# swami1995/diff-qp-mpc

Measured on AMD Instinct MI355X. Metric: QPs/sec (fwd+bwd), batch=4096 n=3 m=3 T=5, higher is better.
Workload: dtype f64; 1 GPU; random dense QP family R (SURVEY 8d), configs[0] shape at the BASELINE metric batch: B=4096/GPU nz=30 nineq=30 neq=15; global_batch=4096, n_state=3, n_ctrl=3, T=5, parallelism=batch-shard x1, termination=batch (the reference's batch-coupled rule, parity-safe)

## Files before the change

diff-qp-mpc_amd/csrc/dqp_r16_prims.h:

```cpp
#ifndef DQP_R16_PRIMS_H_
#define DQP_R16_PRIMS_H_
#include <hip/hip_runtime.h>
#include <math.h>

#include "dqp_common.h"

namespace dqp {
namespace r16 {

template <int CTRL> __device__ __forceinline__ double dppd(double v)
{
    return __builtin_amdgcn_update_dpp(v, v, CTRL, 0xf, 0xf, true);
}

__device__ __forceinline__ double rb(double v, int k)
{
    switch (k & 15) {
    case 0: return dppd<0x150>(v);   case 1: return dppd<0x151>(v);
    case 2: return dppd<0x152>(v);   case 3: return dppd<0x153>(v);
    case 4: return dppd<0x154>(v);   case 5: return dppd<0x155>(v);
    case 6: return dppd<0x156>(v);   case 7: return dppd<0x157>(v);
    case 8: return dppd<0x158>(v);   case 9: return dppd<0x159>(v);
    case 10: return dppd<0x15a>(v);  case 11: return dppd<0x15b>(v);
    case 12: return dppd<0x15c>(v);  case 13: return dppd<0x15d>(v);
// ... 358 lines not shown
            if (16 * s + 15 < k) continue;
            if (16 * s > k) b[s] = fma(-L[s][k], yk, b[s]);
            else b[s] = (r == lk) ? yk : fma(r > lk ? -L[s][k] : 0.0, yk, b[s]);
        }
    }
}

template <int S, int N>
__device__ __forceinline__ void tri_store(double *P, const double (&L)[S][N], int r, double *dummy)
{
#pragma unroll
    for (int s = 0; s < S; ++s) {
        const int i = r + 16 * s;
#pragma unroll
        for (int j = 0; j < N; ++j) {
            if (j > 16 * s + 15) continue;
            double *dst = (i < N && j <= i) ? P + tri(i) + j : dummy;
            *dst = L[s][j];
        }
    }
}

template <int S, int N>
__device__ __forceinline__ void tri_mv(const double *P, const double (&x)[S], double (&y)[S], int r)
{
#pragma unroll
    for (int s = 0; s < S; ++s) y[s] = 0.0;
#pragma unroll
    for (int j = 0; j < N; ++j) {
        const double xb = BC(x, j);
#pragma unroll
        for (int s = 0; s < S; ++s) {
            if (16 * s + 15 < j) continue;
            const int i = r + 16 * s;
            const int ic = i < N ? i : N - 1;
            const double v = P[tri(ic) + (j <= ic ? j : 0)];
            y[s] = fma(mask_hi(v, j <= i && i < N), xb, y[s]);
        }
    }
}

template <int S, int N>
__device__ __forceinline__ void tri_solve(const double *P, const double (&rd)[S], double (&b)[S], int r)
{
#pragma unroll
    for (int k = 0; k < N; ++k) {
        const int sk = k >> 4, lk = k & 15;
        const double yk = rb(b[sk] * rd[sk], lk);
#pragma unroll
        for (int s = 0; s < S; ++s) {
            if (16 * s + 15 < k) continue;
            const int i = r + 16 * s;
            const int ic = i < N ? i : N - 1;
            const double v = P[tri(ic) + (k <= ic ? k : 0)];
            if (16 * s > k) b[s] = fma((i < N) ? -v : 0.0, yk, b[s]);
            else b[s] = (r == lk) ? yk : fma((r > lk && i < N) ? -v : 0.0, yk, b[s]);
        }
    }
}

template <int S, int N>
__device__ __forceinline__ void tri_solve_T(const double *P, const double (&rd)[S], double (&b)[S], int r)
{
#pragma unroll
    for (int j = N - 1; j >= 0; --j) {
        const int sj = j >> 4, lj = j & 15;
        double part = 0.0;
#pragma unroll
        for (int s = 0; s < S; ++s) {
            if (16 * s + 15 <= j) continue;
            const int i = r + 16 * s;
            const int ic = i < N ? i : N - 1;
            const double v = P[tri(ic) + (j <= ic ? j : 0)];
            part = fma((i > j && i < N) ? v : 0.0, b[s], part);
        }
        const double tot = row_sum(part);
        if (r == lj) b[sj] = (b[sj] - tot) * rd[sj];
    }
}

template <int S>
__device__ __forceinline__ void vec_put(double *P, const double (&v)[S], int n, int r, double *dummy)
{
#pragma unroll
    for (int s = 0; s < S; ++s) {
        const int i = r + 16 * s;
        double *dst = i < n ? P + i : dummy;
        *dst = v[s];
    }
}
template <int S>
__device__ __forceinline__ void vec_get(const double *P, double (&v)[S], int n, int r)
{
#pragma unroll
    for (int s = 0; s < S; ++s) {
        const int i = r + 16 * s;
        const double x = P[i < n ? i : n - 1];
        v[s] = i < n ? x : 0.0;
    }
}

template <int S, int NC, bool V2>
__device__ __forceinline__ void load_rows_staged(const double *src, int nrows, double (&dst)[S][NC], int r, double *stage)
{
#pragma unroll
    for (int s = 0; s < S; ++s) {
        const int nr = nrows - 16 * s < 16 ? nrows - 16 * s : 16;
        const double *blk = src + 16 * s * NC;
        if (V2 && (reinterpret_cast<unsigned long long>(blk) & 15ull) == 0) {
            const double2 *b2 = reinterpret_cast<const double2 *>(blk);
            double2 *s2 = reinterpret_cast<double2 *>(stage);
#pragma unroll
            for (int k = 0; k < (16 * NC / 2 + 15) / 16; ++k) {
                const int e = r + 16 * k;
                if (e < nr * NC / 2) s2[e] = b2[e];
            }
            if ((nr * NC) & 1) { if (r == 0) stage[nr * NC - 1] = blk[nr * NC - 1]; }
        } else {
#pragma unroll
            for (int k = 0; k < NC; ++k) {
                const int e = r + 16 * k;
                if (e < nr * NC) stage[e] = blk[e];
            }
        }
        __syncthreads();
        const double *row = stage + (r < nr ? r : 0) * NC;
#pragma unroll
        for (int j = 0; j < NC; ++j) dst[s][j] = row[j];
        if (16 * s + 15 >= nrows) {
            const double keep = r < nr ? 1.0 : 0.0;
#pragma unroll
            for (int j = 0; j < NC; ++j) dst[s][j] *= keep;
        }
        __syncthreads();
    }
}

template <int S, int NC>
__device__ __forceinline__ void load_rows(const double *src, int nrows, double (&dst)[S][NC], int r)
{
#pragma unroll
    for (int s = 0; s < S; ++s) {
        const int i = r + 16 * s;
        const double *row = src + (i < nrows ? i : nrows - 1) * NC;
        const double keep = i < nrows ? 1.0 : 0.0;
#pragma unroll
        for (int j = 0; j < NC; ++j) dst[s][j] = row[j];
        if (16 * s + 15 >= nrows) {
#pragma unroll
            for (int j = 0; j < NC; ++j) dst[s][j] *= keep;
        }
    }
}

template <class C>
__device__ __forceinline__ void load_T(double *lds, double (&T)[C::SM][C::M],
                                       const double (&rdiag)[C::SM], const double (&dinv)[C::SM], int r)
{
    constexpr int M = C::M, SM = C::SM;
    double *Rp = lds + C::oR;
#pragma unroll
    for (int s = 0; s < SM; ++s) {
        const int i = r + 16 * s;
        double *dst = i < M ? Rp + tri(i) + i : lds + C::oDummy + r;
        *dst = rdiag[s] + dinv[s];
    }
#pragma unroll
    for (int s = 0; s < SM; ++s) {
        const int i = r + 16 * s;
        const int ic = i < M ? i : M - 1;
#pragma unroll
        for (int j = 0; j < M; ++j) {
            int off;
            if (16 * s > j) off = tri(ic) + j;
            else if (16 * s + 15 < j) off = tri(j) + ic;
            else off = (j <= ic) ? tri(ic) + j : tri(j) + ic;
            const double v = Rp[off];
            T[s][j] = (16 * s + 15 >= M) ? mask_hi(v, i < M) : v;
        }
    }
}

template <class C>
__device__ __forceinline__ void factor_T(double *lds, double (&T)[C::SM][C::M],
                                         const double (&rdiag)[C::SM], const double (&dinv)[C::SM],
                                         double (&rdu)[C::SM], int r)
{
    load_T<C>(lds, T, rdiag, dinv, r);
    lu_rows<C::SM, C::M>(T, rdu, r);
}

template <class C>
__device__ __forceinline__ void factor_T_rhs(double *lds, double (&T)[C::SM][C::M],
                                             const double (&rdiag)[C::SM], const double (&dinv)[C::SM],
                                             double (&rdu)[C::SM], double (&b)[C::SM], int r)
{
    load_T<C>(lds, T, rdiag, dinv, r);
    lu_factor_solve<C::SM, C::M, DQP_LU_FOLD_RHS != 0>(T, rdu, b, r);
}

}
}
#endif
```

diff-qp-mpc_amd/csrc/dqp_r16n.hip:

```cpp

#include "dqp_r16_prims.h"

namespace dqp {
namespace r16n {

using namespace dqp::r16;

template <int N_, int M_, int E_> struct Cfg {
    static constexpr int N = N_, M = M_, E = E_, R = N_ - E_;
    static constexpr int SN = slots(N_), SM = slots(M_), SR = slots(N_ - E_);
    static constexpr int SE = E_ > 0 ? slots(E_) : 1, EC = E_ > 0 ? E_ : 1;
    static constexpr bool PARK = slots(N_) >= 3;
#ifndef DQP_R16N_PARK_WU
#define DQP_R16N_PARK_WU 1
#endif
    static constexpr bool PARKWU = PARK || DQP_R16N_PARK_WU;
#ifndef DQP_R16N_PIN_ALL
#define DQP_R16N_PIN_ALL 1
#endif
    static constexpr bool PIN = PARK || DQP_R16N_PIN_ALL;
#ifndef DQP_R16N_SPLIT_ALL
#define DQP_R16N_SPLIT_ALL 0
#endif
    static constexpr bool SPLIT = PARK || DQP_R16N_SPLIT_ALL;
#ifndef DQP_R16N_EARLY_CTX
#define DQP_R16N_EARLY_CTX 1
#endif
    static constexpr bool EARLY = DQP_R16N_EARLY_CTX;
    static constexpr int tailsz = E_ * (N_ - E_) + E_ * (E_ - 1) / 2;
    static constexpr int oLq = 0;
    static constexpr int oTl = tri(N_);
    static constexpr int oR = oTl;
    static constexpr int shared = tailsz > tri(M_) ? tailsz : tri(M_);
    static constexpr int oCp = oTl + shared;
    static constexpr int oHp = oCp + (N_ - E_);
    static constexpr int oQv = oHp + M_;
    static constexpr int oBw = oQv + N_;
    static constexpr int oBs = oBw + (N_ - E_), oBz = oBs + M_, oBc = oBz + M_;
    static constexpr int oDummy = oBc + 2;
    static constexpr int ldsQP = oDummy + 16;
    static constexpr int ldsQPpad = (ldsQP + 1) & ~1;
#ifndef DQP_R16N_STAGED
#define DQP_R16N_STAGED 0
#endif
    static constexpr bool STAGED = DQP_R16N_STAGED && 16 * N_ <= ldsQP - oTl;
    __host__ __device__ static constexpr int toff(int k) { return k * (N_ - E_) + k * (k - 1) / 2; }
    static constexpr int wTl = 0, wLq = tailsz, wG = wLq + tri(N_), wU = wG + M_ * N_;
    static constexpr int wTau = wU + E_ * E_, wRdu = wTau + E_, wRdq = wRdu + E_;
    static constexpr int wXy = wRdq + N_, wPy = wXy + E_, wW1 = wPy + E_, wDl = wW1 + E_;
    static constexpr int wsQP = wDl + 1;
    static constexpr int snapDim = (N_ - E_) + 2 * M_ + 2;
};

#define DQP_PHASE_FENCE() asm volatile("" ::: "memory")
__device__ __forceinline__ void pin(double &x) { asm volatile("" : "+v"(x) : : "memory"); }
__device__ __forceinline__ const double *relabel(const double *p)
{
    asm volatile("" : "+v"(p));
    return p;
}

template <class C> struct State {
    double Gh[C::SM][C::N];
    double LqZ[C::SN][C::R];
    double Ah[C::SE][C::N];
    double tau[C::SE];
    double rdu1[C::SE];
    double xy[C::SE];
    double py[C::SE];
    double w1[C::SE];
    double rdq[C::SN];
    double rdiag[C::SM];
    int status;
};

template <class C>
__device__ __forceinline__ void shift_down(const double (&vn)[C::SN], double (&ve)[C::SE], int r)
{
#pragma unroll
    for (int s = 0; s < C::SE; ++s) ve[s] = 0.0;
#pragma unroll
    for (int e = 0; e < C::E; ++e) {
        const double t = BC(vn, C::R + e);
        if (r == (e & 15)) ve[e >> 4] = t;
    }
}
template <class C>
__device__ __forceinline__ void shift_up(const double (&ve)[C::SE], double (&vn)[C::SN], int r)
{
#pragma unroll
    for (int e = 0; e < C::E; ++e) {
        const double t = BC(ve, e);
        if (r == ((C::R + e) & 15)) vn[(C::R + e) >> 4] = t;
    }
}

template <class C>
__device__ __forceinline__ void reflect1(const double *lds, const double (&tau)[C::SE],
                                         double (&v)[C::SN], int k, int r)
{
    const int ck = C::R + k;
    const double *tl = lds + C::oTl + C::toff(k);
    double ud[C::SN], dot = 0.0;
#pragma unroll
    for (int s = 0; s < C::SN; ++s) {
        if (16 * s > ck) { ud[s] = 0.0; continue; }
        const int c = r + 16 * s;
        const double t = tl[c < ck ? c : 0];
        ud[s] = c < ck ? t : (c == ck ? 1.0 : 0.0);
        dot = fma(ud[s], v[s], dot);
    }
    const double tw = BC(tau, k) * row_sum(dot);
#pragma unroll
    for (int s = 0; s < C::SN; ++s)
        if (16 * s <= ck) v[s] = fma(-tw, ud[s], v[s]);
}
template <class C>
__device__ __forceinline__ void apply_QfT(const double *lds, const double (&tau)[C::SE],
                                          double (&v)[C::SN], int r)
{
#pragma unroll
    for (int k = C::E - 1; k >= 0; --k) reflect1<C>(lds, tau, v, k, r);
}
template <class C>
__device__ __forceinline__ void apply_Qf(const double *lds, const double (&tau)[C::SE],
                                         double (&v)[C::SN], int r)
{
#pragma unroll
    for (int k = 0; k < C::E; ++k) reflect1<C>(lds, tau, v, k, r);
}

template <class C>
__device__ __forceinline__ void solve_UT(const State<C> &st, double (&t)[C::SE], int r)
{
#pragma unroll
    for (int j = 0; j < C::E; ++j) {
        const int sj = j >> 4, lj = j & 15;
        double part = 0.0;
#pragma unroll
        for (int s = 0; s < C::SE; ++s) {
            if (16 * s >= j) continue;
            const int k = r + 16 * s;
            part = fma(k < j ? st.Ah[s][C::R + j] : 0.0, t[s], part);
        }
        const double tot = row_sum(part);
        if (r == lj) t[sj] = (t[sj] - tot) * st.rdu1[sj];
    }
}

template <class C>
__device__ __forceinline__ void mul_Gz(const State<C> &st, const double (&v)[C::SR], double (&y)[C::SM])
{
#pragma unroll
    for (int s = 0; s < C::SM; ++s) y[s] = 0.0;
#pragma unroll
    for (int t = 0; t < C::R; ++t) {
        const double vb = BC(v, t);
#pragma unroll
        for (int s = 0; s < C::SM; ++s) y[s] = fma(st.Gh[s][t], vb, y[s]);
    }
}
template <class C>
__device__ __forceinline__ void mul_GzT(const State<C> &st, const double (&v)[C::SM], double (&y)[C::SR], int r)
{
#pragma unroll
    for (int g = 0; g < C::SR; ++g) {
        double p[16];
#pragma unroll
        for (int k = 0; k < 16; ++k) {
            const int c = 16 * g + k;
            if (c < C::R) {
                double a = st.Gh[0][c < C::R ? c : 0] * v[0];
#pragma unroll
                for (int s = 1; s < C::SM; ++s) a = fma(st.Gh[s][c < C::R ? c : 0], v[s], a);
                p[k] = a;
            } else {
                p[k] = 0.0;
            }
        }
        y[g] = reduce_scatter16(p, r);
    }
}
template <class C>
__device__ __forceinline__ void mul_WT(const State<C> &st, const double (&v)[C::SM], double (&y)[C::SE], int r)
{
#pragma unroll
    for (int g = 0; g < C::SE; ++g) {
        double p[16];
#pragma unroll
        for (int k = 0; k < 16; ++k) {
            const int e = 16 * g + k;
            if (e < C::E) {
                double a = st.Gh[0][C::R + (e < C::E ? e : 0)] * v[0];
#pragma unroll
                for (int s = 1; s < C::SM; ++s) a = fma(st.Gh[s][C::R + (e < C::E ? e : 0)], v[s], a);
                p[k] = a;
            } else {
                p[k] = 0.0;
// ... 65 lines not shown
template <int COUNT>
__device__ __forceinline__ void ctx_fetch(const double *src, CtxRegs<COUNT> &t, int r)
{
#pragma unroll
    for (int k = 0; k < (COUNT + 15) / 16; ++k) {
        const int e = r + 16 * k;
        t.v[k] = src[(16 * k + 15 < COUNT || e < COUNT) ? e : COUNT - 1];
    }
}
template <int COUNT>
__device__ __forceinline__ void ctx_stash(double *dst, const CtxRegs<COUNT> &t, int r)
{
#pragma unroll
    for (int k = 0; k < (COUNT + 15) / 16; ++k) {
        const int e = r + 16 * k;
        if (16 * k + 15 < COUNT || e < COUNT) dst[e] = t.v[k];
    }
}
template <int COUNT>
__device__ __forceinline__ void lds_to_ctx(const double *src, double *dst, int r)
{
    CtxRegs<COUNT> t;
    ctx_fetch<COUNT>(src, t, r);
    ctx_stash<COUNT>(dst, t, r);
}

template <class C>
__device__ __forceinline__ void park_GU(double *ws, const State<C> &st, int r)
{
    constexpr int N = C::N, M = C::M, E = C::E, R = C::R;
#pragma unroll
    for (int s = 0; s < C::SM; ++s) {
        const int i = r + 16 * s;
        if (i < M) {
#pragma unroll
            for (int c = 0; c < N; ++c) ws[C::wG + c * M + i] = st.Gh[s][c];
        }
    }
#pragma unroll
    for (int s = 0; s < C::SE; ++s) {
        const int k = r + 16 * s;
        if (k < E) {
#pragma unroll
            for (int e = 0; e < E; ++e) ws[C::wU + e * E + k] = st.Ah[s][R + e];
            ws[C::wTau + k] = st.tau[s];
            ws[C::wRdu + k] = st.rdu1[s];
        }
    }
}
template <class C>
__device__ __forceinline__ void unpark_WU(const double *ws, State<C> &st, int r)
{
    constexpr int M = C::M, E = C::E, R = C::R;
#pragma unroll
    for (int s = 0; s < C::SM; ++s) {
        const int i = r + 16 * s, ic = i < M ? i : M - 1;
#pragma unroll
        for (int e = 0; e < E; ++e) {
            const double v = ws[C::wG + (R + e) * M + ic];
            st.Gh[s][R + e] = i < M ? v : 0.0;
        }
    }
#pragma unroll
    for (int s = 0; s < C::SE; ++s) {
        const int k = r + 16 * s, kc = k < E ? k : E - 1;
#pragma unroll
        for (int e = 0; e < E; ++e) {
            const double v = ws[C::wU + e * E + kc];
            st.Ah[s][R + e] = k < E ? v : 0.0;
        }
    }
}

#ifdef DQP_SETUP_STOP
template <int K, class C> __device__ __forceinline__ double stop_sum(const State<C> &st)
{
    double a = 0.0;
#pragma unroll
    for (int s = 0; s < C::SN; ++s) a += st.rdq[s];
    if (K >= 2 || K == 0) {
#pragma unroll
        for (int s = 0; s < C::SM; ++s)
#pragma unroll
            for (int c = 0; c < C::N; ++c) a += st.Gh[s][c];
#pragma unroll
        for (int s = 0; s < C::SE; ++s)
#pragma unroll
            for (int c = 0; c < C::N; ++c) a += st.Ah[s][c];
    }
    if (K >= 3 || K == 0) {
#pragma unroll
        for (int s = 0; s < C::SE; ++s) a += st.tau[s] + st.rdu1[s] + st.xy[s];
    }
    if (K >= 4 || K == 0) {
#pragma unroll
        for (int s = 0; s < C::SE; ++s) a += st.py[s] + st.w1[s];
    }
    if (K >= 5 || K == 0) {
#pragma unroll
        for (int s = 0; s < C::SN; ++s)
#pragma unroll
            for (int c = 0; c < C::R; ++c) a += st.LqZ[s][c];
    }
    if (K >= 15) {
#pragma unroll
        for (int s = 0; s < C::SM; ++s) a += st.rdiag[s];
    }
    return a;
}
#endif

template <class C>
__device__ __forceinline__ void setup(const KParams &P, long long qp, int r, double *lds, State<C> &st)
{
    constexpr int N = C::N, M = C::M, E = C::E, R = C::R;
    constexpr int SN = C::SN, SM = C::SM, SE = C::SE, SR = C::SR;
    double *dummy = lds + C::oDummy + r;
    st.status = DQP_STATUS_OK;
    double p0[SN], h0[SM], b0[SE];
    const bool mpc = P.mC != nullptr;
    if (mpc) {
        const int n = P.mn, m = P.mm, nt = n + m, T = P.mT;
#pragma unroll
        for (int s = 0; s < SN; ++s) {
            const int i = r + 16 * s, ic = i < N ? i : N - 1, t = ic / nt;
            const double v = P.mc[((long long)t * P.B + qp) * nt + (ic - t * nt)];
            p0[s] = i < N ? v : 0.0;
        }
#pragma unroll
        for (int s = 0; s < SM; ++s) {
            const int i = r + 16 * s, k = (i < T * m ? i : i - T * m), kc = k < T * m ? k : 0, t = kc / m, ju = kc - t * m;
            const long long at = qp * mpc_bound_stride_b(P) + t * mpc_bound_stride_t(P) + ju;
            const double v = i < T * m ? P.muu[at] : -P.mul[at];
            h0[s] = i < M ? v : 0.0;
        }
#pragma unroll
        for (int s = 0; s < SE; ++s) {
            const int e = r + 16 * s, ec = e < E ? e : (E > 0 ? E - 1 : 0), t = ec / n, j = ec - t * n;
            const double v = t < T - 1 ? -P.mf[((long long)t * P.B + qp) * n + j] : P.mx0[qp * n + j];
            b0[s] = (E > 0 && e < E) ? v : 0.0;
        }
    } else {
#pragma unroll
        for (int s = 0; s < SN; ++s) p0[s] = (r + 16 * s < N) ? P.p[qp * P.sp + r + 16 * s] : 0.0;
#pragma unroll
        for (int s = 0; s < SM; ++s) h0[s] = (r + 16 * s < M) ? P.h[qp * P.sh + r + 16 * s] : 0.0;
#pragma unroll
        for (int s = 0; s < SE; ++s) b0[s] = (E > 0 && r + 16 * s < E) ? P.b[qp * P.sb + r + 16 * s] : 0.0;
    }
    {
        double Lq[SN][N];
        if (mpc) mpc_rows_Q<SN, N>(P, qp, Lq, r);
        else if (C::STAGED) load_rows_staged<SN, N, (N * N) % 2 == 0>(P.Q + qp * P.sQ, N, Lq, r, lds + C::oTl);
        else load_rows<SN, N>(P.Q + qp * P.sQ, N, Lq, r);
        if (!chol_rows<SN, N>(Lq, st.rdq, r)) st.status = DQP_STATUS_Q_NOT_PD;
        tri_store<SN, N>(lds + C::oLq, Lq, r, dummy);
    }
    __syncthreads();
    if (C::EARLY) {
        double *ws = P.workspace + qp * (long long)C::wsQP;
        lds_to_ctx<tri(N)>(lds + C::oLq, ws + C::wLq, r);
#pragma unroll
        for (int s = 0; s < SN; ++s)
            if (r + 16 * s < N) ws[C::wRdq + r + 16 * s] = st.rdq[s];
    }
    __builtin_amdgcn_sched_barrier(0);
    DQP_PHASE_FENCE();
    STAMP(P, 1);

    if (mpc) {
        if (!C::SPLIT) mpc_rows_G<SM, N>(P, M, st.Gh, r);
        if (E > 0) mpc_rows_A<SE, N>(P, qp, E, st.Ah, r);
    } else {
        if (C::STAGED) {
            if (!C::SPLIT) load_rows_staged<SM, N, (M * N) % 2 == 0>(P.G + qp * P.sG, M, st.Gh, r, lds + C::oTl);
            if (E > 0) load_rows_staged<SE, N, (C::EC * N) % 2 == 0>(P.A + qp * P.sA, E, st.Ah, r, lds + C::oTl);
        } else {
            if (!C::SPLIT) load_rows<SM, N>(P.G + qp * P.sG, M, st.Gh, r);
            if (E > 0) load_rows<SE, N>(P.A + qp * P.sA, E, st.Ah, r);
        }
    }
    {
        const double *Lp = lds + C::oLq;
#pragma unroll
        for (int j = 0; j < N; ++j) {
#pragma unroll
            for (int k = 0; k < j; ++k) {
                const double ljk = Lp[tri(j) + k];
                if (!C::SPLIT) {
#pragma unroll
                    for (int s = 0; s < SM; ++s) st.Gh[s][j] = fma(-st.Gh[s][k], ljk, st.Gh[s][j]);
                }
                if (E > 0) {
#pragma unroll
                    for (int s = 0; s < SE; ++s) st.Ah[s][j] = fma(-st.Ah[s][k], ljk, st.Ah[s][j]);
                }
            }
            const double rj = BC(st.rdq, j);
            if (!C::SPLIT) {
#pragma unroll
                for (int s = 0; s < SM; ++s) st.Gh[s][j] *= rj;
            }
            if (E > 0) {
#pragma unroll
                for (int s = 0; s < SE; ++s) st.Ah[s][j] *= rj;
            }
            if (C::PIN) {
#pragma unroll
                for (int s = 0; s < SE; ++s) pin(st.Ah[s][j]);
                if (!C::SPLIT) {
#pragma unroll
                    for (int s = 0; s < SM; ++s) pin(st.Gh[s][j]);
                }
            }
            __builtin_amdgcn_sched_barrier(0);
        }
    }
    __builtin_amdgcn_sched_barrier(0);
    DQP_PHASE_FENCE();
    STAMP(P, 2);

#pragma unroll
    for (int s = 0; s < SE; ++s) { st.tau[s] = 0.0; st.rdu1[s] = 0.0; st.xy[s] = 0.0; st.py[s] = 0.0; st.w1[s] = 0.0; }

    if (E > 0) {
        double nmax = 0.0;
#pragma unroll
        for (int k = E - 1; k >= 0; --k) {
            const int sk = k >> 4, lk = k & 15, ck = R + k;
#ifdef DQP_STAMPS_C
            if (k < 15) { STAMPC(P, k); }
#endif
            double u[N];
            double nrm2 = 0.0;
#pragma unroll
            for (int c = 0; c <= ck; ++c) {
                u[c] = rb(st.Ah[sk][c], lk);
                nrm2 = fma(u[c], u[c], nrm2);
            }
            if (!(nrm2 > 1e-26 * nmax)) { if (st.status == DQP_STATUS_OK) st.status = DQP_STATUS_A_RANK_DEF; nrm2 = 1.0; }
            nmax = fmax(nmax, nrm2);
            const double vk = u[ck];
            const double alpha = -copysign(sqrt(nrm2), vk);
            const double uck = vk - alpha;
            const double iu = frcp(uck);
            const double tauk = uck * uck * frcp(nrm2 - alpha * vk);
            double *tl = lds + C::oTl + C::toff(k);
            if (C::PIN) {
#pragma unroll
                for (int c = 0; c < ck; ++c) u[c] *= iu;
                if (r == 0) {
#pragma unroll
                    for (int c = 0; c < ck; ++c) tl[c] = u[c];
                }
            } else {
#pragma unroll
                for (int c = 0; c < ck; ++c) {
                    u[c] *= iu;
                    double *dst = (r == 0) ? tl + c : dummy;
                    *dst = u[c];
                }
            }
            if (r == lk) { st.tau[sk] = tauk; st.rdu1[sk] = frcp(alpha); }
#pragma unroll
            for (int s = 0; s < SE; ++s) {
                if (16 * s > k) continue;
                double w = st.Ah[s][ck];
#pragma unroll
                for (int c = 0; c < ck; ++c) w = fma(st.Ah[s][c], u[c], w);
                double tw = tauk * w;
                if (16 * s + 15 >= k) tw = (r + 16 * s < k) ? tw : 0.0;
#pragma unroll
                for (int c = 0; c < ck; ++c) st.Ah[s][c] = fma(-tw, u[c], st.Ah[s][c]);
                st.Ah[s][ck] -= tw;
            }
            if (r == lk) st.Ah[sk][ck] = alpha;
            if (!C::SPLIT) {
#pragma unroll
                for (int s = 0; s < SM; ++s) {
                    double w = st.Gh[s][ck];
#pragma unroll
                    for (int c = 0; c < ck; ++c) w = fma(st.Gh[s][c], u[c], w);
                    const double tw = tauk * w;
#pragma unroll
                    for (int c = 0; c < ck; ++c) st.Gh[s][c] = fma(-tw, u[c], st.Gh[s][c]);
                    st.Gh[s][ck] -= tw;
                }
            }
            if (C::PIN) {
#pragma unroll
                for (int s = 0; s < SE; ++s) pin(st.Ah[s][ck]);
                if (!C::SPLIT) {
#pragma unroll
                    for (int s = 0; s < SM; ++s) pin(st.Gh[s][ck]);
                }
            }
        }
#ifdef DQP_STAMPS_C
        STAMPC(P, 15);
#endif
        __syncthreads();
        __builtin_amdgcn_sched_barrier(0);
        if (C::EARLY) {
            double *ws = P.workspace + qp * (long long)C::wsQP;
            lds_to_ctx<C::tailsz>(lds + C::oTl, ws + C::wTl, r);
        }
        DQP_PHASE_FENCE();

        {
            double b[SE];
#pragma unroll
            for (int s = 0; s < SE; ++s) b[s] = b0[s];
#pragma unroll
            for (int j = E - 1; j >= 0; --j) {
                const int sj = j >> 4, lj = j & 15;
                const double xj = rb(b[sj] * st.rdu1[sj], lj);
#pragma unroll
                for (int s = 0; s < SE; ++s) {
                    if (16 * s > j) continue;
                    const int k = r + 16 * s;
                    b[s] = (k == j) ? xj : fma(k < j ? -st.Ah[s][R + j] : 0.0, xj, b[s]);
                }
            }
#pragma unroll
            for (int s = 0; s < SE; ++s) st.xy[s] = b[s];
        }
    }
    __builtin_amdgcn_sched_barrier(0);
    DQP_PHASE_FENCE();
// ... 353 lines not shown
            s_[s] = -z[s];
            ms = fmin(ms, inM[s] ? s_[s] : INFINITY);
            mz = fmin(mz, inM[s] ? z[s] : INFINITY);
        }
        ms = row_min(ms); mz = row_min(mz);
#pragma unroll
        for (int s = 0; s < SM; ++s) {
            if (ms < 0.0 && inM[s]) s_[s] -= ms - 1.0;
            if (mz < 0.0 && inM[s]) z[s] -= mz - 1.0;
        }
        delta = mz < 0.0 ? 1.0 - mz : 0.0;
        if (r == 0) P.workspace[qp * (long long)C::wsQP + C::wDl] = delta;
    }

    double gz[SR];
    mul_GzT<C>(st, z, gz, r);
    STAMP(P, 6);
    double best = INFINITY, bestc = 1.0;
    bool have_best = false, done = false;
    int nNot = 0, iters = 0;

    if (maxIter > 0) for (int it = 0;; ++it) {
        double rw[SR], rz[SM];
        {
            double cp[SR], hp[SM], gw[SM];
            vec_get<SR>(lds + C::oCp, cp, R, r);
            vec_get<SM>(lds + C::oHp, hp, M, r);
            mul_Gz<C>(st, w, gw);
#pragma unroll
            for (int s = 0; s < SR; ++s) rw[s] = inR[s] ? w[s] + cp[s] + gz[s] : 0.0;
#pragma unroll
            for (int s = 0; s < SM; ++s) rz[s] = inM[s] ? gw[s] + s_[s] - hp[s] : 0.0;
        }
        double sz = 0.0, nz2 = 0.0;
#pragma unroll
        for (int s = 0; s < SM; ++s) { sz = fma(s_[s], z[s], sz); nz2 = fma(rz[s], rz[s], nz2); }
        double nx2 = rx_norm2_partial<C>(st, lds, rw, cc * delta, r);
        sz = row_sum(sz); nz2 = row_sum(nz2); nx2 = row_sum(nx2);
        const double mu = fabs(sz * (1.0 / M));
        const double resid = sqrt(nz2) + sqrt(nx2) + M * mu;
        if (!done) {
            iters = it + 1;
            if (!have_best || resid < best) {
                nNot = 0; have_best = true; best = resid; bestc = cc;
                vec_put<SR>(lds + C::oBw, w, R, r, dummy);
                vec_put<SM>(lds + C::oBs, s_, M, r, dummy);
                vec_put<SM>(lds + C::oBz, z, M, r, dummy);
                if (P.snap && live) {
                    double *sp = P.snap + ((long long)it * P.B + qp) * C::snapDim;
#pragma unroll
                    for (int s = 0; s < SR; ++s)
                        if (inR[s]) sp[r + 16 * s] = w[s];
#pragma unroll
                    for (int s = 0; s < SM; ++s)
                        if (inM[s]) { sp[R + r + 16 * s] = s_[s]; sp[R + M + r + 16 * s] = z[s]; }
                    if (r == 0) sp[R + 2 * M] = cc;
                }
            } else {
                nNot += 1;
            }
            if (batch) {
                if (P.hist && r == 0 && live) hist_put(P, qp, it, resid, mu);
                done = !(fabs(resid) < INFINITY);
            } else if ((nNot >= P.notImprovedLim && best < P.stallTol) || best < P.eps || mu > 1e32 ||
                       !(fabs(resid) < INFINITY))
                done = true;
        }
        if (__builtin_amdgcn_ballot_w64(!done) == 0 || it + 1 >= maxIter) break;
        if (it == 1) STAMP(P, 9);

        double dza[SM], dsa[SM];
        {
            double gu[SM];
            mul_Gz<C>(st, rw, gu);
#pragma unroll
            for (int s = 0; s < SM; ++s) dza[s] = rz[s] - s_[s] - gu[s];
        }
        __builtin_amdgcn_sched_barrier(0);
        double dinv[SM];
#pragma unroll
        for (int s = 0; s < SM; ++s) dinv[s] = inM[s] ? s_[s] * frcp(z[s]) : 0.0;
        factor_T_rhs<C>(lds, T, st.rdiag, dinv, rdu, dza, r);
        if (it == 1) STAMP(P, 10);
        if (it == 1) STAMP(P, 11);
        double rzv[SM], rsv[SM];
#pragma unroll
        for (int s = 0; s < SM; ++s) {
            rzv[s] = inM[s] ? frcp(z[s]) : 0.0;
            rsv[s] = inM[s] ? frcp(s_[s]) : 0.0;
        }
        double tm = 0.0;
#pragma unroll
        for (int s = 0; s < SM; ++s) {
            dsa[s] = (-z[s] - dza[s]) * dinv[s];
            tm = fmax(tm, fmax(-dza[s] * rzv[s], -dsa[s] * rsv[s]));
        }
        bool zero_step = false;
        if (strict) {
#pragma unroll
            for (int s = 0; s < SM; ++s) zero_step |= inM[s] && (dza[s] == 0.0 || dsa[s] == 0.0);
        }
        double alpha = frcp(fmax(row_max(tm), 1.0));
        double t3 = 0.0;
#pragma unroll
        for (int s = 0; s < SM; ++s)
            t3 = fma(fma(alpha, dsa[s], s_[s]), fma(alpha, dza[s], z[s]), t3);
        t3 = row_sum(t3);
        double sig = t3 / sz;
        sig = sig * sig * sig;
        double rsc[SM], dzc[SM], dz[SM], ds[SM];
#pragma unroll
        for (int s = 0; s < SM; ++s) {
            rsc[s] = fma(dsa[s], dza[s], -mu * sig) * rsv[s];
            dzc[s] = -rsc[s] * dinv[s];
        }
        lu_solve<SM, M>(T, rdu, dzc, r);
        if (it == 1) STAMP(P, 12);
        tm = 0.0;
#pragma unroll
        for (int s = 0; s < SM; ++s) {
            dz[s] = dza[s] + dzc[s];
            ds[s] = fma(-rsc[s] - dzc[s], dinv[s], dsa[s]);
            tm = fmax(tm, fmax(-dz[s] * rzv[s], -ds[s] * rsv[s]));
        }
        if (strict) {
#pragma unroll
            for (int s = 0; s < SM; ++s) zero_step |= inM[s] && (dz[s] == 0.0 || ds[s] == 0.0);
            if ((__builtin_amdgcn_ballot_w64(zero_step) >> (lane & 48)) & 0xffffull) done = true;
        }
        __builtin_amdgcn_sched_barrier(0);
        double gtd[SR];
        mul_GzT<C>(st, dz, gtd, r);
        alpha = frcp(fmax(row_max(tm) * (1.0 / 0.999), 1.0));
        if (!done) {
#pragma unroll
            for (int s = 0; s < SR; ++s) {
                w[s] = fma(alpha, -rw[s] - gtd[s], w[s]);
                gz[s] = fma(alpha, gtd[s], gz[s]);
            }
#pragma unroll
            for (int s = 0; s < SM; ++s) { s_[s] = fma(alpha, ds[s], s_[s]); z[s] = fma(alpha, dz[s], z[s]); }
            cc *= (1.0 - alpha);
        }
        if (it == 1) STAMP(P, 13);
        if (it == 0) STAMP(P, 8);
    }
    STAMP(P, 7);

    if (P.hist && r == 0 && live) hist_fill(P, qp, iters);
    epilogue<C>(P, qp, r, lds, st, bestc, delta, iters, best, live, true);
    STAMP(P, 14);
}

template <class C>
__device__ __forceinline__ void load_ctx(const KParams &P, long long qp, int r, double *lds, State<C> &st)
{
    constexpr int N = C::N, M = C::M, E = C::E, R = C::R;
    constexpr int SN = C::SN, SM = C::SM, SE = C::SE;
    st.status = DQP_STATUS_OK;
    {
        const double *ws = P.workspace + qp * (long long)C::wsQP;
        CtxRegs<C::tailsz> tl;
        CtxRegs<tri(N)> lq;
        ctx_fetch<C::tailsz>(ws + C::wTl, tl, r);
        ctx_fetch<tri(N)>(ws + C::wLq, lq, r);
        ctx_stash<C::tailsz>(lds + C::oTl, tl, r);
        ctx_stash<tri(N)>(lds + C::oLq, lq, r);
#pragma unroll
        for (int s = 0; s < SM; ++s) {
            const int i = r + 16 * s, ic = i < M ? i : M - 1;
#pragma unroll
            for (int c = 0; c < N; ++c) {
                const double v = ws[C::wG + c * M + ic];
                st.Gh[s][c] = (16 * s + 15 >= M) ? mask_hi(v, i < M) : v;
            }
        }
#pragma unroll
        for (int s = 0; s < SE; ++s) {
            const int k = r + 16 * s, kc = k < E ? k : E - 1;
#pragma unroll
            for (int c = 0; c < N; ++c) st.Ah[s][c] = 0.0;
#pragma unroll
            for (int e = 0; e < E; ++e) {
                const double v = ws[C::wU + e * E + kc];
                st.Ah[s][R + e] = k < E ? v : 0.0;
            }
            const double t = ws[C::wTau + kc], u = ws[C::wRdu + kc];
            st.tau[s] = k < E ? t : 0.0;
            st.rdu1[s] = k < E ? u : 0.0;
        }
#pragma unroll
        for (int s = 0; s < SN; ++s) {
            const int i = r + 16 * s;
            const double v = ws[C::wRdq + (i < N ? i : N - 1)];
            st.rdq[s] = i < N ? v : 0.0;
        }
    }
}

template <class C>
__global__ __launch_bounds__(64) void finish_kernel(KParams P)
{
    constexpr int M = C::M, E = C::E, R = C::R;
    constexpr int SM = C::SM, SE = C::SE, SR = C::SR;
    extern __shared__ __attribute__((aligned(16))) double sm[];
    const int lane = threadIdx.x, r = lane & 15, qrow = lane >> 4;
    long long qp = (long long)blockIdx.x * 4 + qrow;
    bool live = qp < P.B;
    if (!live) qp = P.B - 1;
    live = live && term_flagged(P, qp);
    if (__builtin_amdgcn_ballot_w64(live) == 0) return;
    const int cap = min(P.maxIter, P.cap[0]);
    double *lds = sm + qrow * C::ldsQPpad;
    double *dummy = lds + C::oDummy + r;
    State<C> st;
    load_ctx<C>(P, qp, r, lds, st);
    const double *ws = P.workspace + qp * (long long)C::wsQP;
#pragma unroll
    for (int s = 0; s < SE; ++s) {
        const int k = r + 16 * s, kc = k < E ? k : (E > 0 ? E - 1 : 0);
        const double a = ws[C::wXy + kc], b = ws[C::wPy + kc], c = ws[C::wW1 + kc];
        st.xy[s] = (E > 0 && k < E) ? a : 0.0;
        st.py[s] = (E > 0 && k < E) ? b : 0.0;
        st.w1[s] = (E > 0 && k < E) ? c : 0.0;
    }
    const double delta = ws[C::wDl];
    const double2 *h = reinterpret_cast<const double2 *>(P.histIn) + qp;
    double hv[64];
#pragma unroll
    for (int it = 0; it < 64; ++it) hv[it] = h[(long long)(it < cap ? it : 0) * P.B].x;
    double best = hv[0];
    int arg = 0;
#pragma unroll
    for (int it = 1; it < 64; ++it)
        if (it < cap && hv[it] < best) { best = hv[it]; arg = it; }
    const double *sp = P.snap + ((long long)arg * P.B + qp) * C::snapDim;
    double bw[SR], bs[SM], bz[SM];
#pragma unroll
    for (int s = 0; s < SR; ++s) { const int i = r + 16 * s; const double v = sp[i < R ? i : 0]; bw[s] = i < R ? v : 0.0; }
#pragma unroll
    for (int s = 0; s < SM; ++s) {
        const int i = r + 16 * s, ic = i < M ? i : 0;
        const double a = sp[R + ic], b = sp[R + M + ic];
        bs[s] = i < M ? a : 0.0;
        bz[s] = i < M ? b : 0.0;
    }
    const double bestc = sp[R + 2 * M];
    vec_put<SR>(lds + C::oBw, bw, R, r, dummy);
    vec_put<SM>(lds + C::oBs, bs, M, r, dummy);
    vec_put<SM>(lds + C::oBz, bz, M, r, dummy);
    st.status = P.info ? P.info[2 * qp] : DQP_STATUS_OK;
    epilogue<C>(P, qp, r, lds, st, bestc, delta, cap, best, live, false);
}

template <class C>
__global__ __launch_bounds__(64) void backward_kernel(KParams P)
{
    constexpr int N = C::N, M = C::M, E = C::E, R = C::R;
    constexpr int SN = C::SN, SM = C::SM, SE = C::SE, SR = C::SR;
    extern __shared__ __attribute__((aligned(16))) double sm[];
    const int lane = threadIdx.x, r = lane & 15, qrow = lane >> 4;
    long long qp = (long long)blockIdx.x * 4 + qrow;
    const bool live = qp < P.B;
    if (!live) qp = P.B - 1;
    double *lds = sm + qrow * C::ldsQPpad;

    State<C> st;
    load_ctx<C>(P, qp, r, lds, st);
    __syncthreads();

    bool inN[SN], inM[SM], inE[SE];
#pragma unroll
    for (int s = 0; s < SN; ++s) inN[s] = r + 16 * s < N;
#pragma unroll
    for (int s = 0; s < SM; ++s) inM[s] = r + 16 * s < M;
#pragma unroll
    for (int s = 0; s < SE; ++s) inE[s] = r + 16 * s < E;

    double zh[SN], g[SN], lam[SM], dinv[SM], nu[SE];
#pragma unroll
    for (int s = 0; s < SN; ++s) {
        zh[s] = inN[s] ? P.zin[qp * N + r + 16 * s] : 0.0;
        g[s] = inN[s] ? P.gin[qp * N + r + 16 * s] : 0.0;
    }
#pragma unroll
    for (int s = 0; s < SM; ++s) {
        lam[s] = inM[s] ? P.lamin[qp * M + r + 16 * s] : 0.0;
        const double sl = inM[s] ? P.slackin[qp * M + r + 16 * s] : 1.0;
        if (P.flags & DQP_FLAG_DENSE_BACKWARD) dinv[s] = inM[s] ? sl / lam[s] : 0.0;
        else dinv[s] = inM[s] ? fmax(sl, 1e-8) / fmax(lam[s], 1e-8) : 0.0;
    }
#pragma unroll
    for (int s = 0; s < SE; ++s) nu[s] = (E > 0 && inE[s]) ? P.nuin[qp * E + r + 16 * s] : 0.0;

    tri_solve<SN, N>(lds + C::oLq, st.rdq, g, r);
    double gy[SE];
#pragma unroll
    for (int s = 0; s < SE; ++s) gy[s] = 0.0;
    if (E > 0) {
        apply_QfT<C>(lds, st.tau, g, r);
        shift_down<C>(g, gy, r);
    }
    double gz[SR];
#pragma unroll
    for (int s = 0; s < SR; ++s) gz[s] = (r + 16 * s < R) ? g[s] : 0.0;

    double dlam[SM];
    mul_Gz<C>(st, gz, dlam);
#pragma unroll
    for (int s = 0; s < SM; ++s) dlam[s] = -dlam[s];
    __builtin_amdgcn_sched_barrier(0);
    {
        double T[SM][M], rdu[SM];
#pragma unroll
        for (int j = 0; j < M; ++j) {
            const int sj = j >> 4, lj = j & 15;
            double acc[SM];
#pragma unroll
            for (int s = 0; s < SM; ++s) acc[s] = (r + 16 * s == j) ? dinv[s] : 0.0;
#pragma unroll
            for (int c = 0; c < R; ++c) {
                const double gb = rb(st.Gh[sj][c], lj);
#pragma unroll
                for (int s = 0; s < SM; ++s) acc[s] = fma(st.Gh[s][c], gb, acc[s]);
            }
#pragma unroll
            for (int s = 0; s < SM; ++s) T[s][j] = acc[s];
            __builtin_amdgcn_sched_barrier(0);
        }
        lu_factor_solve<SM, M, DQP_LU_FOLD_RHS != 0>(T, rdu, dlam, r);
    }
    __builtin_amdgcn_sched_barrier(0);
    double dxh[SN], dnu[SE];
    {
        double gtd[SR];
        mul_GzT<C>(st, dlam, gtd, r);
#pragma unroll
        for (int s = 0; s < SN; ++s) dxh[s] = (s < SR && r + 16 * s < R) ? -(gz[s < SR ? s : 0] + gtd[s < SR ? s : 0]) : 0.0;
    }
#pragma unroll
    for (int s = 0; s < SE; ++s) dnu[s] = 0.0;
    if (E > 0) {
        apply_Qf<C>(lds, st.tau, dxh, r);
        double wz[SE];
        mul_WT<C>(st, dlam, wz, r);
#pragma unroll
        for (int s = 0; s < SE; ++s) dnu[s] = inE[s] ? -(gy[s] + wz[s]) : 0.0;
        solve_UT<C>(st, dnu, r);
    }
    tri_solve_T<SN, N>(lds + C::oLq, st.rdq, dxh, r);

    if (!live) return;
    if (P.mdc || P.mdC || P.mdF || P.mdf || P.mdx0) {
        const int n = P.mn, m = P.mm, nt = n + m, T = P.mT;
        const long long Bq = P.B;
        int tl[SN], jl[SN];
#pragma unroll
        for (int s = 0; s < SN; ++s) { const int c = r + 16 * s; tl[s] = c / nt; jl[s] = c - tl[s] * nt; }
        if (P.mdc) {
#pragma unroll
            for (int s = 0; s < SN; ++s)
                if (inN[s]) P.mdc[((long long)tl[s] * Bq + qp) * nt + jl[s]] = dxh[s];
        }
        if (P.mdC) {
            int ti = 0, ji = 0;
#pragma unroll
            for (int i = 0; i < N; ++i) {
                const double dxi = BC(dxh, i), zi = BC(zh, i);
#pragma unroll
                for (int s = 0; s < SN; ++s)
                    if (inN[s] && tl[s] == ti)
                        P.mdC[(((long long)ti * Bq + qp) * nt + ji) * nt + jl[s]] = 0.5 * (dxi * zh[s] + zi * dxh[s]);
                if (++ji == nt) { ji = 0; ++ti; }
            }
        }
        if (E > 0) {
            int te = 0, je = 0;
#pragma unroll
            for (int e = 0; e < E; ++e) {
                const double dni = BC(dnu, e), ni = BC(nu, e);
                if (te < T - 1) {
                    if (P.mdF) {
#pragma unroll
                        for (int s = 0; s < SN; ++s)
                            if (inN[s] && tl[s] == te)
                                P.mdF[(((long long)te * Bq + qp) * n + je) * nt + jl[s]] = dni * zh[s] + ni * dxh[s];
                    }
                    if (P.mdf && r == 0) P.mdf[((long long)te * Bq + qp) * n + je] = dni;
                } else if (P.mdx0 && r == 0) {
                    P.mdx0[qp * n + je] = -dni;
                }
                if (++je == n) { je = 0; ++te; }
            }
        }
        if (r == 0 && P.info) { P.info[2 * qp] = st.status; P.info[2 * qp + 1] = 0; }
        return;
    }
#pragma unroll
    for (int s = 0; s < SN; ++s)
        if (P.dp && inN[s]) P.dp[qp * N + r + 16 * s] = dxh[s];
#pragma unroll
    for (int s = 0; s < SM; ++s)
        if (P.dh && inM[s]) P.dh[qp * M + r + 16 * s] = -dlam[s];
    if (E > 0) {
#pragma unroll
        for (int s = 0; s < SE; ++s)
            if (P.db && inE[s]) P.db[qp * E + r + 16 * s] = -dnu[s];
    }
    if (P.dQ) {
        double *o = P.dQ + qp * N * N;
#pragma unroll
        for (int i = 0; i < N; ++i) {
            const double dxi = BC(dxh, i), zi = BC(zh, i);
#pragma unroll
            for (int s = 0; s < SN; ++s)
                if (inN[s]) o[i * N + r + 16 * s] = 0.5 * (dxi * zh[s] + zi * dxh[s]);
        }
    }
    if (P.dG) {
        double *o = P.dG + qp * M * N;
#pragma unroll
        for (int i = 0; i < M; ++i) {
            const double dli = BC(dlam, i), li = BC(lam, i);
#pragma unroll
            for (int s = 0; s < SN; ++s)
                if (inN[s]) o[i * N + r + 16 * s] = dli * zh[s] + li * dxh[s];
        }
    }
    if (P.dA && E > 0) {
        double *o = P.dA + qp * E * N;
#pragma unroll
        for (int i = 0; i < E; ++i) {
            const double dni = BC(dnu, i), ni = BC(nu, i);
#pragma unroll
            for (int s = 0; s < SN; ++s)
                if (inN[s]) o[i * N + r + 16 * s] = dni * zh[s] + ni * dxh[s];
        }
    }
    if (r == 0 && P.info) { P.info[2 * qp] = st.status; P.info[2 * qp + 1] = 0; }
}

template <class C, class K>
int launch(K kernel, const KParams &P, void *stream)
{
    const size_t lds = (size_t)4 * C::ldsQPpad * sizeof(double);
    if (lds > 64 * 1024 &&
        hipFuncSetAttribute(reinterpret_cast<const void *>(kernel),
                            hipFuncAttributeMaxDynamicSharedMemorySize, (int)lds) != hipSuccess)
        return DQP_ERR_LAUNCH;
    const int blocks = (P.B + 3) / 4;
    DQP_LAUNCH(kernel, dim3(blocks), dim3(64), lds, (hipStream_t)stream, P);
    return hipGetLastError() == hipSuccess ? DQP_OK : DQP_ERR_LAUNCH;
}

}

#if !defined(DQP_R16_N) || !defined(DQP_R16_M) || !defined(DQP_R16_E)
#error "compile with -DDQP_R16_N=.. -DDQP_R16_M=.. -DDQP_R16_E=.."
#endif
#define DQP_CAT2(a, n, m, e) a##n##_##m##_##e
#define DQP_CAT(a, n, m, e) DQP_CAT2(a, n, m, e)

#ifndef DQP_R16_BWD
int DQP_CAT(r16n_forward_, DQP_R16_N, DQP_R16_M, DQP_R16_E)(const KParams &P, void *stream)
{
    using C = r16n::Cfg<DQP_R16_N, DQP_R16_M, DQP_R16_E>;
    if (P.cap && P.snap && P.histIn) return r16n::launch<C>(r16n::finish_kernel<C>, P, stream);
    return r16n::launch<C>(r16n::forward_kernel<C>, P, stream);
}
#else
int DQP_CAT(r16n_backward_, DQP_R16_N, DQP_R16_M, DQP_R16_E)(const KParams &P, void *stream)
{
    using C = r16n::Cfg<DQP_R16_N, DQP_R16_M, DQP_R16_E>;
    return r16n::launch<C>(r16n::backward_kernel<C>, P, stream);
}
#endif

}
```

Before: 17.51 million QPs/sec.

## Issue G/A and context loads early to overlap memory latency with compute

In the forward context setup, G and A rows are now loaded right after Q rows, so their memory latency overlaps the Cholesky factorisation, and masking is applied later. In the backward kernel, the workspace context loads (triangular factors, G columns, U, tau, rdu) are split into issue and finish stages. They are issued alongside the per-QP input loads, and masking and LDS stashing are deferred until just before each piece is consumed. This aims to hide global-load latency, at the cost of higher register pressure and more complex barrier and fence ordering.

```diff
diff --git a/diff-qp-mpc_amd/csrc/dqp_r16_prims.h b/diff-qp-mpc_amd/csrc/dqp_r16_prims.h
--- a/diff-qp-mpc_amd/csrc/dqp_r16_prims.h
+++ b/diff-qp-mpc_amd/csrc/dqp_r16_prims.h
@@ -534,6 +534,29 @@
         }
     }
 }
+template <int S, int NC>
+__device__ __forceinline__ void load_rows_issue(const double *src, int nrows, double (&dst)[S][NC], int r)
+{
+#pragma unroll
+    for (int s = 0; s < S; ++s) {
+        const int i = r + 16 * s;
+        const double *row = src + (i < nrows ? i : nrows - 1) * NC;
+#pragma unroll
+        for (int j = 0; j < NC; ++j) dst[s][j] = row[j];
+    }
+}
+template <int S, int NC>
+__device__ __forceinline__ void load_rows_mask(int nrows, double (&dst)[S][NC], int r)
+{
+#pragma unroll
+    for (int s = 0; s < S; ++s) {
+        const double keep = r + 16 * s < nrows ? 1.0 : 0.0;
+        if (16 * s + 15 >= nrows) {
+#pragma unroll
+            for (int j = 0; j < NC; ++j) dst[s][j] *= keep;
+        }
+    }
+}
 
 template <class C>
 __device__ __forceinline__ void load_T(double *lds, double (&T)[C::SM][C::M],
diff --git a/diff-qp-mpc_amd/csrc/dqp_r16n.hip b/diff-qp-mpc_amd/csrc/dqp_r16n.hip
--- a/diff-qp-mpc_amd/csrc/dqp_r16n.hip
+++ b/diff-qp-mpc_amd/csrc/dqp_r16n.hip
@@ -44,6 +44,10 @@
 #define DQP_R16N_STAGED 0
 #endif
     static constexpr bool STAGED = DQP_R16N_STAGED && 16 * N_ <= ldsQP - oTl;
+#ifndef DQP_R16N_EARLY_GA
+#define DQP_R16N_EARLY_GA 1
+#endif
+    static constexpr bool EARLYGA = DQP_R16N_EARLY_GA && !SPLIT && !STAGED;
     __host__ __device__ static constexpr int toff(int k) { return k * (N_ - E_) + k * (k - 1) / 2; }
     static constexpr int wTl = 0, wLq = tailsz, wG = wLq + tri(N_), wU = wG + M_ * N_;
     static constexpr int wTau = wU + E_ * E_, wRdu = wTau + E_, wRdq = wRdu + E_;
@@ -415,7 +419,13 @@
         double Lq[SN][N];
         if (mpc) mpc_rows_Q<SN, N>(P, qp, Lq, r);
         else if (C::STAGED) load_rows_staged<SN, N, (N * N) % 2 == 0>(P.Q + qp * P.sQ, N, Lq, r, lds + C::oTl);
-        else load_rows<SN, N>(P.Q + qp * P.sQ, N, Lq, r);
+        else {
+            load_rows<SN, N>(P.Q + qp * P.sQ, N, Lq, r);
+            if (C::EARLYGA) {
+                load_rows_issue<SM, N>(P.G + qp * P.sG, M, st.Gh, r);
+                if (E > 0) load_rows_issue<SE, N>(P.A + qp * P.sA, E, st.Ah, r);
+            }
+        }
         if (!chol_rows<SN, N>(Lq, st.rdq, r)) st.status = DQP_STATUS_Q_NOT_PD;
         tri_store<SN, N>(lds + C::oLq, Lq, r, dummy);
     }
@@ -438,6 +448,9 @@
         if (C::STAGED) {
             if (!C::SPLIT) load_rows_staged<SM, N, (M * N) % 2 == 0>(P.G + qp * P.sG, M, st.Gh, r, lds + C::oTl);
             if (E > 0) load_rows_staged<SE, N, (C::EC * N) % 2 == 0>(P.A + qp * P.sA, E, st.Ah, r, lds + C::oTl);
+        } else if (C::EARLYGA) {
+            load_rows_mask<SM, N>(M, st.Gh, r);
+            if (E > 0) load_rows_mask<SE, N>(E, st.Ah, r);
         } else {
             if (!C::SPLIT) load_rows<SM, N>(P.G + qp * P.sG, M, st.Gh, r);
             if (E > 0) load_rows<SE, N>(P.A + qp * P.sA, E, st.Ah, r);
@@ -1097,50 +1110,101 @@
     STAMP(P, 14);
 }
 
+template <class C> struct CtxA {
+    CtxRegs<C::tailsz> tl;
+    CtxRegs<tri(C::N)> lq;
+};
+#ifndef DQP_R16N_BWD_ORDERED_CTX
+#define DQP_R16N_BWD_ORDERED_CTX 1
+#endif
+template <class C>
+__device__ __forceinline__ void ctx_issue_a(const double *ws, int r, CtxA<C> &a, State<C> &st)
+{
+    ctx_fetch<C::tailsz>(ws + C::wTl, a.tl, r);
+    ctx_fetch<tri(C::N)>(ws + C::wLq, a.lq, r);
+#pragma unroll
+    for (int s = 0; s < C::SN; ++s) {
+        const int i = r + 16 * s;
+        st.rdq[s] = ws[C::wRdq + (i < C::N ? i : C::N - 1)];
+    }
+#pragma unroll
+    for (int s = 0; s < C::SE; ++s) {
+        const int k = r + 16 * s;
+        st.tau[s] = ws[C::wTau + (k < C::E ? k : C::E - 1)];
+    }
+}
+template <class C>
+__device__ __forceinline__ void ctx_finish_a(double *lds, int r, const CtxA<C> &a, State<C> &st)
+{
+    ctx_stash<C::tailsz>(lds + C::oTl, a.tl, r);
+    ctx_stash<tri(C::N)>(lds + C::oLq, a.lq, r);
+#pragma unroll
+    for (int s = 0; s < C::SN; ++s) st.rdq[s] = r + 16 * s < C::N ? st.rdq[s] : 0.0;
+#pragma unroll
+    for (int s = 0; s < C::SE; ++s) st.tau[s] = r + 16 * s < C::E ? st.tau[s] : 0.0;
+}
+template <class C, int C0, int C1>
+__device__ __forceinline__ void ctx_issue_G(const double *ws, int r, State<C> &st)
+{
+#pragma unroll
+    for (int s = 0; s < C::SM; ++s) {
+        const int i = r + 16 * s, ic = i < C::M ? i : C::M - 1;
+#pragma unroll
+        for (int c = C0; c < C1; ++c) st.Gh[s][c] = ws[C::wG + c * C::M + ic];
+    }
+}
+template <class C, int C0, int C1>
+__device__ __forceinline__ void ctx_finish_G(int r, State<C> &st)
+{
+#pragma unroll
+    for (int s = 0; s < C::SM; ++s) {
+        if (16 * s + 15 < C::M) continue;
+#pragma unroll
+        for (int c = C0; c < C1; ++c) st.Gh[s][c] = mask_hi(st.Gh[s][c], r + 16 * s < C::M);
+    }
+}
+template <class C>
+__device__ __forceinline__ void ctx_issue_c(const double *ws, int r, State<C> &st)
+{
+    ctx_issue_G<C, C::R, C::N>(ws, r, st);
+#pragma unroll
+    for (int s = 0; s < C::SE; ++s) {
+        const int k = r + 16 * s, kc = k < C::E ? k : C::E - 1;
+#pragma unroll
+        for (int e = 0; e < C::E; ++e) st.Ah[s][C::R + e] = ws[C::wU + e * C::E + kc];
+        st.rdu1[s] = ws[C::wRdu + kc];
+    }
+}
+template <class C>
+__device__ __forceinline__ void ctx_finish_c(int r, State<C> &st)
+{
+    ctx_finish_G<C, C::R, C::N>(r, st);
+#pragma unroll
+    for (int s = 0; s < C::SE; ++s) {
+        const bool in = r + 16 * s < C::E;
+#pragma unroll
+        for (int e = 0; e < C::E; ++e) st.Ah[s][C::R + e] = in ? st.Ah[s][C::R + e] : 0.0;
+        st.rdu1[s] = in ? st.rdu1[s] : 0.0;
+    }
+}
 template <class C>
 __device__ __forceinline__ void load_ctx(const KParams &P, long long qp, int r, double *lds, State<C> &st)
 {
-    constexpr int N = C::N, M = C::M, E = C::E, R = C::R;
-    constexpr int SN = C::SN, SM = C::SM, SE = C::SE;
     st.status = DQP_STATUS_OK;
+    const double *ws = P.workspace + qp * (long long)C::wsQP;
+#pragma unroll
+    for (int s = 0; s < C::SE; ++s)
+#pragma unroll
+        for (int c = 0; c < C::R; ++c) st.Ah[s][c] = 0.0;
     {
-        const double *ws = P.workspace + qp * (long long)C::wsQP;
-        CtxRegs<C::tailsz> tl;
-        CtxRegs<tri(N)> lq;
-        ctx_fetch<C::tailsz>(ws + C::wTl, tl, r);
-        ctx_fetch<tri(N)>(ws + C::wLq, lq, r);
-        ctx_stash<C::tailsz>(lds + C::oTl, tl, r);
-        ctx_stash<tri(N)>(lds + C::oLq, lq, r);
-#pragma unroll
-        for (int s = 0; s < SM; ++s) {
-            const int i = r + 16 * s, ic = i < M ? i : M - 1;
-#pragma unroll
-            for (int c = 0; c < N; ++c) {
-                const double v = ws[C::wG + c * M + ic];
-                st.Gh[s][c] = (16 * s + 15 >= M) ? mask_hi(v, i < M) : v;
-            }
-        }
-#pragma unroll
-        for (int s = 0; s < SE; ++s) {
-            const int k = r + 16 * s, kc = k < E ? k : E - 1;
-#pragma unroll
-            for (int c = 0; c < N; ++c) st.Ah[s][c] = 0.0;
-#pragma unroll
-            for (int e = 0; e < E; ++e) {
-                const double v = ws[C::wU + e * E + kc];
-                st.Ah[s][R + e] = k < E ? v : 0.0;
-            }
-            const double t = ws[C::wTau + kc], u = ws[C::wRdu + kc];
-            st.tau[s] = k < E ? t : 0.0;
-            st.rdu1[s] = k < E ? u : 0.0;
-        }
-#pragma unroll
-        for (int s = 0; s < SN; ++s) {
-            const int i = r + 16 * s;
-            const double v = ws[C::wRdq + (i < N ? i : N - 1)];
-            st.rdq[s] = i < N ? v : 0.0;
-        }
-    }
+        CtxA<C> a;
+        ctx_issue_a<C>(ws, r, a, st);
+        ctx_finish_a<C>(lds, r, a, st);
+    }
+    ctx_issue_G<C, 0, C::R>(ws, r, st);
+    ctx_issue_c<C>(ws, r, st);
+    ctx_finish_G<C, 0, C::R>(r, st);
+    ctx_finish_c<C>(r, st);
 }
 
 template <class C>
@@ -1210,19 +1274,30 @@
     if (!live) qp = P.B - 1;
     double *lds = sm + qrow * C::ldsQPpad;
 
+    bool inN[SN], inM[SM], inE[SE];
+#pragma unroll
+    for (int s = 0; s < SN; ++s) inN[s] = r + 16 * s < N;
+#pragma unroll
+    for (int s = 0; s < SM; ++s) inM[s] = r + 16 * s < M;
+#pragma unroll
+    for (int s = 0; s < SE; ++s) inE[s] = r + 16 * s < E;
+
+    constexpr bool ORD = DQP_R16N_BWD_ORDERED_CTX && !C::PARK;
     State<C> st;
-    load_ctx<C>(P, qp, r, lds, st);
-    __syncthreads();
-
-    bool inN[SN], inM[SM], inE[SE];
-#pragma unroll
-    for (int s = 0; s < SN; ++s) inN[s] = r + 16 * s < N;
-#pragma unroll
-    for (int s = 0; s < SM; ++s) inM[s] = r + 16 * s < M;
-#pragma unroll
-    for (int s = 0; s < SE; ++s) inE[s] = r + 16 * s < E;
-
-    double zh[SN], g[SN], lam[SM], dinv[SM], nu[SE];
+    const double *ws = P.workspace + qp * (long long)C::wsQP;
+    double zh[SN], g[SN], lam[SM], sl[SM], dinv[SM], nu[SE];
+    if (ORD) {
+        st.status = DQP_STATUS_OK;
+#pragma unroll
+        for (int s = 0; s < SE; ++s)
+#pragma unroll
+            for (int c = 0; c < R; ++c) st.Ah[s][c] = 0.0;
+    } else {
+        load_ctx<C>(P, qp, r, lds, st);
+        __syncthreads();
+    }
+    CtxA<C> ca;
+    if (ORD) ctx_issue_a<C>(ws, r, ca, st);
 #pragma unroll
     for (int s = 0; s < SN; ++s) {
         zh[s] = inN[s] ? P.zin[qp * N + r + 16 * s] : 0.0;
@@ -1231,12 +1306,24 @@
 #pragma unroll
     for (int s = 0; s < SM; ++s) {
         lam[s] = inM[s] ? P.lamin[qp * M + r + 16 * s] : 0.0;
-        const double sl = inM[s] ? P.slackin[qp * M + r + 16 * s] : 1.0;
-        if (P.flags & DQP_FLAG_DENSE_BACKWARD) dinv[s] = inM[s] ? sl / lam[s] : 0.0;
-        else dinv[s] = inM[s] ? fmax(sl, 1e-8) / fmax(lam[s], 1e-8) : 0.0;
+        sl[s] = inM[s] ? P.slackin[qp * M + r + 16 * s] : 1.0;
     }
 #pragma unroll
     for (int s = 0; s < SE; ++s) nu[s] = (E > 0 && inE[s]) ? P.nuin[qp * E + r + 16 * s] : 0.0;
+    if (ORD) {
+        ctx_issue_G<C, 0, R>(ws, r, st);
+        ctx_issue_c<C>(ws, r, st);
+        __builtin_amdgcn_sched_barrier(0);
+        ctx_finish_a<C>(lds, r, ca, st);
+        __builtin_amdgcn_fence(__ATOMIC_RELEASE, "workgroup", "local");
+        __builtin_amdgcn_s_barrier();
+        __builtin_amdgcn_fence(__ATOMIC_ACQUIRE, "workgroup", "local");
+    }
+#pragma unroll
+    for (int s = 0; s < SM; ++s) {
+        if (P.flags & DQP_FLAG_DENSE_BACKWARD) dinv[s] = inM[s] ? sl[s] / lam[s] : 0.0;
+        else dinv[s] = inM[s] ? fmax(sl[s], 1e-8) / fmax(lam[s], 1e-8) : 0.0;
+    }
 
     tri_solve<SN, N>(lds + C::oLq, st.rdq, g, r);
     double gy[SE];
@@ -1251,6 +1338,12 @@
     for (int s = 0; s < SR; ++s) gz[s] = (r + 16 * s < R) ? g[s] : 0.0;
 
     double dlam[SM];
+    if (ORD) {
+#pragma unroll
+        for (int s = 0; s < SR; ++s) pin(gz[s]);
+        __builtin_amdgcn_sched_barrier(0);
+        ctx_finish_G<C, 0, R>(r, st);
+    }
     mul_Gz<C>(st, gz, dlam);
 #pragma unroll
     for (int s = 0; s < SM; ++s) dlam[s] = -dlam[s];
@@ -1287,6 +1380,10 @@
     for (int s = 0; s < SE; ++s) dnu[s] = 0.0;
     if (E > 0) {
         apply_Qf<C>(lds, st.tau, dxh, r);
+        if (ORD) {
+            __builtin_amdgcn_sched_barrier(0);
+            ctx_finish_c<C>(r, st);
+        }
         double wz[SE];
         mul_WT<C>(st, dlam, wz, r);
 #pragma unroll
```

Measured after the change: 17.16 million QPs/sec. -2.0%, worse.
